# genjax-community/genjax

Measured on AMD Instinct MI355X. Metric: particle_steps_per_sec, higher is better.
Workload: dtype f32; 1 GPU; gmm_c8_d16 ImportanceK: propagate+reweight+LSE, systematic resample, gather (BASELINE.json configs[1]); k_particles_per_gpu=1048576, k_particles_total=1048576, rng_stream=flat, exchange=none

## Files before the change

### genjax_amd/csrc/gjx_resample.hip

```cpp
#include <math.h>
#include <string.h>

#include "gjx_device.h"
#include "gjx_host.h"
#include "gjx_scan.h"
#include "gjx_tile.h"

namespace gjx {

struct PickPair {
  float v;
  int32_t i;
};

GJX_DEV void pick_better(float& v, int32_t& i, float ov, int32_t oi) {
  if (ov > v || (ov == v && oi < i)) { v = ov; i = oi; }
}

template <int RNG>
__global__ __launch_bounds__(256) void k_pick_partial(const float* logw, int64_t K, int64_t offset, const float* lse,
                                                     key2 key, PickPair* partials) {
  __shared__ float rv[4];
  __shared__ int32_t ri[4];
  const float l = lse[2];
  float bv = -INFINITY;
  int32_t bi = 0x7FFFFFFF;
  for (int64_t i = (int64_t)blockIdx.x * 256 + threadIdx.x; i < K; i += (int64_t)gridDim.x * 256) {
    const uint64_t gi = (uint64_t)(offset + i);
    uint32_t bits;
    if (RNG == GJX_RNG_JAX32) {
      const key2 h = fold_in64(key, gi);
      bits = h.a ^ h.b;
    } else {
      const key2 h = fold_in64(key, gi >> 1);
      bits = (gi & 1u) ? h.b : h.a;
    }
    const float v = (logw[i] - l) + gumbel_from_bits(bits);
    pick_better(bv, bi, v, (int32_t)gi);
  }
#pragma unroll
  for (int o = 32; o > 0; o >>= 1) {
    const float ov = __shfl_xor(bv, o, 64);
    const int32_t oi = __shfl_xor(bi, o, 64);
    pick_better(bv, bi, ov, oi);
  }
  if ((threadIdx.x & 63) == 0) { rv[threadIdx.x >> 6] = bv; ri[threadIdx.x >> 6] = bi; }
  __syncthreads();
  if (threadIdx.x == 0) {
    for (int w = 1; w < 4; ++w) pick_better(bv, bi, rv[w], ri[w]);
    partials[blockIdx.x] = PickPair{bv, bi};
  }
}

__global__ __launch_bounds__(256) void k_pick_finish(const PickPair* partials, int n, PickPair* out) {
  __shared__ float rv[4];
  __shared__ int32_t ri[4];
  float bv = -INFINITY;
// ... 182 lines not shown
        const int h = atomicAdd(&n_heavy, 1);
        h_i[h] = (int32_t)i; h_lo[h] = lo; h_hi[h] = hi;
      } else if (hi > lo) {
        if (ancestors) for (int64_t j = lo; j < hi; ++j) ancestors[j] = (int32_t)i;
        if (GATHER) {
          for (int r = 0; r < rows; ++r) {
            const float v = src[(int64_t)r * src_stride + i];
            for (int64_t j = lo; j < hi; ++j) dst[(int64_t)r * dst_stride + j] = v;
          }
        }
      }
    }
  }
  __syncthreads();
  const int nh = n_heavy;
  for (int h = 0; h < nh; ++h) {
    const int32_t pi = h_i[h];
    const int64_t lo = h_lo[h], hi = h_hi[h];
    if (ancestors) for (int64_t j = lo + threadIdx.x; j < hi; j += 256) ancestors[j] = pi;
    if (GATHER) {
      for (int r = 0; r < rows; ++r) {
        const float v = src[(int64_t)r * src_stride + pi];
        for (int64_t j = lo + threadIdx.x; j < hi; j += 256) dst[(int64_t)r * dst_stride + j] = v;
      }
    }
  }
}

template <int ITEMS>
__global__ __launch_bounds__(256) void k_resample_fused(const float* __restrict__ x, int64_t K, int mode,
                                                       const float* lse, int n_partials, float* lse_out,
                                                       float log_k_total, double u, int64_t N, int32_t* ancestors,
                                                       uint64_t* cum_out, uint64_t* base_total_out,
                                                       unsigned long long* agg, unsigned* ctrl) {
  __shared__ float fred[8];
  __shared__ ScanSmem sm;
  unsigned epoch;
  const unsigned long long tag = grid_tag(ctrl, &epoch);
  const int64_t i0 = ((int64_t)blockIdx.x * 256 + threadIdx.x) * ITEMS;
  float xv[ITEMS];
#pragma unroll
  for (int k = 0; k < ITEMS; ++k) xv[k] = (i0 + k < K) ? x[i0 + k] : 0.0f;
  float sm_sum;
  const float mx = block_ref_max(mode, lse, n_partials, fred, &sm_sum);
  if (mode == 2 && lse_out && blockIdx.x == 0 && threadIdx.x == 0) {
    const float l = mx > -INFINITY ? mx + logf(sm_sum) : -INFINITY;
    lse_out[0] = mx; lse_out[1] = sm_sum; lse_out[2] = l; lse_out[3] = l - log_k_total;
  }
  tile_scan_expand<ITEMS, false>(xv, mode, mx, i0, K, u, N, ancestors, cum_out, base_total_out, agg, tag, ctrl, epoch, true, sm);
}

constexpr int kGatherMaxTiles = 1024;

template <int ITEMS>
__global__ __launch_bounds__(256) void k_resample_gather(const float* __restrict__ x, int64_t K, int mode,
                                                        const float* lse, int n_partials, float* lse_out,
                                                        float log_k_total, double u, const float* __restrict__ src,
                                                        int64_t src_stride, int rows, float* __restrict__ dst,
                                                        int64_t dst_stride, int32_t* ancestors,
                                                        unsigned long long* agg, unsigned* ctrl,
                                                        unsigned long long* timeline) {
#define GJX_STAMP(n) do { if (timeline && threadIdx.x == 0) timeline[blockIdx.x * 8 + (n)] = __builtin_amdgcn_s_memrealtime(); } while (0)
  GJX_STAMP(0);
  constexpr int TILE = 256 * ITEMS;
  __shared__ float fred[8];
  __shared__ uint64_t wsum[4];
  __shared__ uint64_t P[kGatherMaxTiles + 1];
  constexpr int CH = 3;
  __shared__ uint64_t cumL[CH * TILE];
  __shared__ uint64_t s_wtot[CH][4];
  __shared__ int s_range[2];
  unsigned epoch;
  const unsigned long long tag = grid_tag(ctrl, &epoch);
  const int nb = (int)gridDim.x;
  const int lane = threadIdx.x & 63, wid = threadIdx.x >> 6;
  const int64_t i0 = ((int64_t)blockIdx.x * 256 + threadIdx.x) * ITEMS;
  auto load_tile = [&](int64_t p0, float (&v)[ITEMS]) {
    if (ITEMS == 4 && p0 + 4 <= K) {
      const float4 q4 = *(const float4*)(x + p0);
      v[0] = q4.x; v[1] = q4.y; v[2] = q4.z; v[3] = q4.w;
    } else {
#pragma unroll
      for (int k = 0; k < ITEMS; ++k) v[k] = (p0 + k < K) ? x[p0 + k] : 0.0f;
    }
  };
  const int w0 = (int)blockIdx.x - 1;
  float xv[ITEMS], xn[2][ITEMS];
  load_tile(i0, xv);
  float sm_sum;
  const float mx = block_ref_max(mode, lse, n_partials, fred, &sm_sum);
  if (mode == 2 && lse_out && blockIdx.x == 0 && threadIdx.x == 0) {
    const float l = mx > -INFINITY ? mx + logf(sm_sum) : -INFINITY;
    lse_out[0] = mx; lse_out[1] = sm_sum; lse_out[2] = l; lse_out[3] = l - log_k_total;
  }
  uint64_t qown[ITEMS], sown = 0, incown;
  {
#pragma unroll
    for (int k = 0; k < ITEMS; ++k) { sown += (i0 + k < K) ? weight_q(xv, k, mode, mx) : 0; qown[k] = sown; }
    incown = wave_scan_u64(sown);
    if (lane == 63) { wsum[wid] = incown; s_wtot[1][wid] = incown; }
    __syncthreads();
    if (threadIdx.x == 0) grid_publish(agg, tag, wsum[0] + wsum[1] + wsum[2] + wsum[3]);
  }
  GJX_STAMP(1);
#pragma unroll
  for (int c = 0; c < 2; ++c) {
    const int tc = w0 + 2 * c;
#pragma unroll
    for (int k = 0; k < ITEMS; ++k) xn[c][k] = 0.0f;
    if (tc >= 0 && tc < nb) load_tile((int64_t)tc * TILE + (int64_t)threadIdx.x * ITEMS, xn[c]);
  }
  {
    uint64_t qn[2][ITEMS], sn[2], incn[2];
#pragma unroll
// ... 131 lines not shown
        inc[c] = sacc[c];
      }
#pragma unroll
      for (int c = 0; c < CH; ++c) inc[c] = wave_scan_u64(inc[c]);
      if (lane == 63) {
#pragma unroll
        for (int c = 0; c < CH; ++c) s_wtot[c][wid] = inc[c];
      }
      __syncthreads();
#pragma unroll
      for (int c = 0; c < CH; ++c) {
        uint64_t base = P[tsrc[c]] + (inc[c] - sacc[c]);
        for (int w = 0; w < wid; ++w) base += s_wtot[c][w];
#pragma unroll
        for (int k = 0; k < ITEMS; ++k) cumL[c * TILE + threadIdx.x * ITEMS + k] = base + qi[c][k];
      }
      __syncthreads();
      int pos[ITEMS];
      const uint64_t* cm[ITEMS];
      bool mine[ITEMS];
#pragma unroll
      for (int k = 0; k < ITEMS; ++k) {
        mine[k] = kpos[k] >= idx && kpos[k] < idx + CH;
        cm[k] = cumL + (mine[k] ? (kpos[k] - idx) * TILE : 0);
        pos[k] = 0;
      }
#pragma unroll
      for (int q = TILE >> 2; q >= 1; q >>= 2) {
#pragma unroll
        for (int k = 0; k < ITEMS; ++k) {
          const uint64_t pa = cm[k][pos[k] + q - 1], pb = cm[k][pos[k] + 2 * q - 1], pc = cm[k][pos[k] + 3 * q - 1];
          pos[k] += (pa <= T[k] ? q : 0) + (pb <= T[k] ? q : 0) + (pc <= T[k] ? q : 0);
        }
      }
#pragma unroll
      for (int k = 0; k < ITEMS; ++k)
        if (mine[k]) anc[k] = (int32_t)((int64_t)tile[k] * TILE + pos[k]);
      idx = nidx;
    }
    }
  }
  GJX_STAMP(4);
#pragma unroll
  for (int k = 0; k < ITEMS; ++k) anc[k] = max(0, min(anc[k], (int32_t)(K - 1)));
  const bool whole = i0 + ITEMS <= K;
  if (ancestors) {
    if (ITEMS == 4 && whole) *(int4*)(ancestors + i0) = make_int4(anc[0], anc[1], anc[2], anc[3]);
    else {
#pragma unroll
      for (int k = 0; k < ITEMS; ++k) if (i0 + k < K) ancestors[i0 + k] = anc[k];
    }
  }
  const bool vec = ITEMS == 4 && whole && (dst_stride & 3) == 0 && (((uintptr_t)dst) & 15) == 0;
  if (vec) {
#pragma unroll 4
    for (int r = 0; r < rows; ++r) {
      const float* sr = src + (int64_t)r * src_stride;
      float4 v;
      v.x = sr[anc[0]]; v.y = sr[anc[ITEMS > 1 ? 1 : 0]]; v.z = sr[anc[ITEMS > 2 ? 2 : 0]]; v.w = sr[anc[ITEMS > 3 ? 3 : 0]];
      *(float4*)(dst + (int64_t)r * dst_stride + i0) = v;
    }
  } else {
#pragma unroll 4
    for (int r = 0; r < rows; ++r) {
      const float* sr = src + (int64_t)r * src_stride;
#pragma unroll
      for (int k = 0; k < ITEMS; ++k) if (i0 + k < K) dst[(int64_t)r * dst_stride + i0 + k] = sr[anc[k]];
    }
  }
  GJX_STAMP(5);
#undef GJX_STAMP
}

constexpr int kGatherTiledMaxTiles = 65536;

template <bool GATED>
__global__ __launch_bounds__(kTileQ) void k_tile_totals(const float* __restrict__ logw, int64_t K, uint64_t* S, int32_t* E, const int32_t* gate) {
  constexpr int NW = kTileQ / 64;
  if (GATED && *gate == 0) return;
  __shared__ float fred[NW];
  __shared__ uint64_t wsum[NW];
  const int lane = threadIdx.x & 63, wid = threadIdx.x >> 6;
  const int64_t i = (int64_t)blockIdx.x * kTileQ + threadIdx.x;
  const float lw = i < K ? logw[i] : -INFINITY;
  const float wm = wave_max(lw);
  if (lane == 0) fred[wid] = wm;
  __syncthreads();
  float bm = fred[0];
#pragma unroll
  for (int w = 1; w < NW; ++w) bm = fmaxf(bm, fred[w]);
  const int e = tile_exponent(bm);
  const uint64_t tot_w = wave_total_u64(i < K ? tile_q(lw, e) : 0);
  if (lane == 0) wsum[wid] = tot_w;
  __syncthreads();
  if (threadIdx.x == 0) {
    uint64_t tot = 0;
    for (int w = 0; w < NW; ++w) tot += wsum[w];
    S[blockIdx.x] = tot;
    E[blockIdx.x] = tot ? e : kTileDead;
  }
}

template <int ITEMS, bool PLANNED, bool GATED>
__global__ __launch_bounds__(256) void k_resample_gather_tiled(const float* __restrict__ x, int64_t K, const uint64_t* __restrict__ S,
                                                              const int32_t* __restrict__ E, const uint64_t* __restrict__ Pg,
                                                              const int32_t* __restrict__ shg, int lse_mode, const float* lse,
                                                              int n_partials, float* lse_out, float log_k_total, double u,
                                                              const float* __restrict__ src, int64_t src_stride, int rows,
                                                              float* __restrict__ dst, int64_t dst_stride, int32_t* ancestors,
                                                              unsigned* ctrl, unsigned long long* timeline, const int32_t* gate) {
#define GJX_STAMP(n) do { if (timeline && threadIdx.x == 0) timeline[blockIdx.x * 8 + (n)] = __builtin_amdgcn_s_memrealtime(); } while (0)
  GJX_STAMP(0);
  static_assert(ITEMS == 4, "a block consumes one quantisation tile: 256 lanes x 4 slots");
  extern __shared__ __align__(16) unsigned char gt_dyn[];
  const int nt = (int)gridDim.x;
  uint64_t* const Pl = (uint64_t*)gt_dyn;
  int32_t* const Ebl = (int32_t*)(Pl + ((nt + 2) & ~1));
  __shared__ TiledSearchShared sh;
  const int64_t i0 = ((int64_t)blockIdx.x * 256 + threadIdx.x) * ITEMS;
  int32_t anc[ITEMS];
  if (GATED && *gate == 0) {
#pragma unroll
    for (int k = 0; k < ITEMS; ++k) anc[k] = (int32_t)((i0 + k < K) ? i0 + k : K - 1);
  } else
  tiled_search_tile<PLANNED>(x, K, S, E, Pg, shg, nt, (int)blockIdx.x, Pl, Ebl, sh, lse_mode, lse, n_partials, lse_out, log_k_total, u, ctrl, timeline, anc);
  GJX_STAMP(4);
  const bool whole = i0 + ITEMS <= K;
  if (ancestors) {
    if (whole) *(int4*)(ancestors + i0) = make_int4(anc[0], anc[1], anc[2], anc[3]);
    else {
#pragma unroll
      for (int k = 0; k < ITEMS; ++k) if (i0 + k < K) ancestors[i0 + k] = anc[k];
    }
  }
  const bool vec = whole && (dst_stride & 3) == 0 && (((uintptr_t)dst) & 15) == 0;
  if (vec) {
#pragma unroll 4
    for (int r = 0; r < rows; ++r) {
      const float* sr = src + (int64_t)r * src_stride;
      float4 v;
      v.x = sr[anc[0]]; v.y = sr[anc[1]]; v.z = sr[anc[2]]; v.w = sr[anc[3]];
      *(float4*)(dst + (int64_t)r * dst_stride + i0) = v;
    }
  } else {
#pragma unroll 4
    for (int r = 0; r < rows; ++r) {
      const float* sr = src + (int64_t)r * src_stride;
#pragma unroll
      for (int k = 0; k < ITEMS; ++k) if (i0 + k < K) dst[(int64_t)r * dst_stride + i0 + k] = sr[anc[k]];
    }
  }
  GJX_STAMP(5);
#undef GJX_STAMP
}

__global__ __launch_bounds__(256) void k_multinomial(const uint64_t* cum, int64_t K, const uint64_t* base_total,
                                                    key2 key, int64_t out_begin, int64_t n_out, int32_t* ancestors) {
  const int64_t j = (int64_t)blockIdx.x * 256 + threadIdx.x;
  if (j >= n_out) return;
  const uint64_t base = base_total[0], total = base_total[1];
  const key2 h = fold_in64(key, (uint64_t)(out_begin + j));
  const uint64_t r = (((uint64_t)h.a << 32) | h.b) >> 11;
  const double uj = (double)r * (1.0 / 9007199254740992.0);
  const uint64_t T = (uint64_t)(uj * (double)total);
  int32_t a = -1;
  if (K > 0) {
    const uint64_t local = cum[K - 1];
    if (T >= base && T < base + local) a = (int32_t)upper_search(cum, K, T - base);
  }
  ancestors[j] = a;
}

__global__ __launch_bounds__(256) void k_gather_rows(const float* __restrict__ src, int64_t src_stride,
                                                    const int32_t* __restrict__ anc, int64_t n_out, int rows,
                                                    float* __restrict__ dst, int64_t dst_stride) {
  const int64_t j = (int64_t)blockIdx.x * 256 + threadIdx.x;
  if (j >= n_out) return;
  const int32_t a = anc[j];
  if ((uint64_t)(int64_t)a >= (uint64_t)src_stride) return;
  for (int r = 0; r < rows; ++r) dst[(int64_t)r * dst_stride + j] = src[(int64_t)r * src_stride + a];
}


int launch_expand_planned(const uint64_t* cum, int64_t K, const gjx_shard_plan* plan_dev, double u, int64_t N_total,
                          int32_t* ancestors, int64_t anc_capacity, hipStream_t st) {
  const uint64_t* bt = reinterpret_cast<const uint64_t*>(plan_dev);
  const int64_t* range = reinterpret_cast<const int64_t*>(plan_dev) + 2;
  hipLaunchKernelGGL(k_systematic_expand<false>, dim3((unsigned)((K + 255) / 256)), dim3(256), 0, st, cum, K, bt, u, N_total,
                     (int64_t)0, anc_capacity, ancestors, (const float*)nullptr, (int64_t)0, 0, (float*)nullptr, (int64_t)0,
                     range);
  GJX_CHECK_LAUNCH("gjx_shard_resample(expand)");
  return GJX_OK;
}

struct EssArgs {
  const float* inc;
  float* W;
  float* w_copy;
  int64_t K;
  const int32_t* fresh;
  unsigned long long* pm;
  unsigned* p2;
  unsigned* ticket;
  float* out4;
// ... 157 lines not shown
  GJX_CHECK_LAUNCH("gjx_categorical_pick/partial");
  hipLaunchKernelGGL(k_pick_finish, dim3(1), dim3(256), 0, st, (const PickPair*)partials, nblocks, (PickPair*)out_dev);
  GJX_CHECK_LAUNCH("gjx_categorical_pick/finish");
  return GJX_OK;
}

extern "C" int gjx_trials_lse_pick(const float* logw, int64_t n_trials, int64_t K, int64_t particle_offset, uint32_t key0, uint32_t key1,
                                   int32_t rng_mode, float* lse_out, int32_t* pick_out, void* stream) {
  if (!logw || !lse_out || n_trials <= 0 || K <= 0 || n_trials > 0x7fffffffLL || particle_offset < 0 ||
      (pick_out && particle_offset + n_trials * K > 0x7fffffffLL))
    return gjx_fail(GJX_EINVAL, "gjx_trials_lse_pick: bad argument");
  hipStream_t st = (hipStream_t)stream;
  const float log_k = (float)log((double)K);
  if (rng_mode == GJX_RNG_JAX32)
    hipLaunchKernelGGL(k_trials_lse_pick<GJX_RNG_JAX32>, dim3((unsigned)n_trials), dim3(256), 0, st, logw, K, particle_offset, key2{key0, key1},
                       pick_out ? 1 : 0, log_k, lse_out, pick_out);
  else
    hipLaunchKernelGGL(k_trials_lse_pick<GJX_RNG_FLAT>, dim3((unsigned)n_trials), dim3(256), 0, st, logw, K, particle_offset, key2{key0, key1},
                       pick_out ? 1 : 0, log_k, lse_out, pick_out);
  GJX_CHECK_LAUNCH("gjx_trials_lse_pick");
  return GJX_OK;
}

extern "C" int gjx_weight_cumsum(const float* x, int64_t K, int32_t is_log, const float* lse, int32_t n_partials,
                                 uint64_t* cum, uint64_t* base_total_dev, float* lse_out, int64_t K_total,
                                 void* workspace, size_t workspace_bytes, void* stream) {
  if (!x || !cum || !base_total_dev || K <= 0 || is_log < 0 || is_log > 2 || (is_log && !lse) || (is_log == 2 && n_partials <= 0))
    return gjx_fail(GJX_EINVAL, "gjx_weight_cumsum: bad argument");
  if (!workspace || workspace_bytes < gjx_workspace_bytes(GJX_OP_RESAMPLE, K)) return gjx_fail(GJX_EWORKSPACE, "gjx_weight_cumsum: workspace too small");
  hipStream_t st = (hipStream_t)stream;
  const int nblocks = (int)((K + kScanTile - 1) / kScanTile);
  uint64_t* bs = (uint64_t*)((char*)workspace + kWsHeaderBytes);
  const float log_k = (float)log((double)(K_total > 0 ? K_total : K));
  hipLaunchKernelGGL(k_wsum_blocks, dim3(nblocks), dim3(256), 0, st, x, K, (int)is_log, lse, (int)n_partials, lse_out, log_k, bs);
  GJX_CHECK_LAUNCH("gjx_weight_cumsum/sum");
  hipLaunchKernelGGL(k_wscan_write, dim3(nblocks), dim3(256), 0, st, x, K, (int)is_log, lse, (int)n_partials, (const uint64_t*)bs, cum, base_total_dev);
  GJX_CHECK_LAUNCH("gjx_weight_cumsum/write");
  return GJX_OK;
}

extern "C" int gjx_resample_systematic(const uint64_t* cum, int64_t K, const uint64_t* base_total_dev, double u,
                                       int64_t N_total, int64_t out_begin, int64_t n_out, int32_t* ancestors,
                                       void* stream) {
  if (!cum || !base_total_dev || !ancestors || K <= 0 || N_total <= 0 || n_out < 0 || !(u >= 0.0 && u < 1.0))
    return gjx_fail(GJX_EINVAL, "gjx_resample_systematic: bad argument");
  if (n_out == 0) return GJX_OK;
  hipLaunchKernelGGL(k_systematic_expand<false>, dim3((unsigned)((K + 255) / 256)), dim3(256), 0, (hipStream_t)stream, cum, K,
                     base_total_dev, u, N_total, out_begin, n_out, ancestors, (const float*)nullptr, (int64_t)0, 0,
                     (float*)nullptr, (int64_t)0);
  GJX_CHECK_LAUNCH("gjx_resample_systematic");
  return GJX_OK;
}

static int env_items() {
  const char* e = getenv("GJX_RESAMPLE_ITEMS");
  const int v = e ? atoi(e) : 0;
  return (v == 1 || v == 4 || v == 16) ? v : 0;
}

extern "C" int gjx_resample_indices(const float* x, int64_t K, int32_t is_log, const float* lse, int32_t n_partials,
                                    double u, int64_t N, int32_t* ancestors, uint64_t* cum, uint64_t* base_total_dev,
                                    float* lse_out, int64_t K_total, void* workspace, size_t workspace_bytes, void* stream) {
  if (!x || K <= 0 || N <= 0 || is_log < 0 || is_log > 2 || (is_log && !lse) || (is_log == 2 && n_partials <= 0) ||
      !(u >= 0.0 && u < 1.0) || (!ancestors && !cum))
    return gjx_fail(GJX_EINVAL, "gjx_resample_indices: bad argument");
  if (!workspace || workspace_bytes < gjx_workspace_bytes(GJX_OP_RESAMPLE, K)) return gjx_fail(GJX_EWORKSPACE, "gjx_resample_indices: workspace too small");
  int items = env_items();
  int64_t nblocks = 0;
  const int cand[3] = {1, 4, 16};
  bool fits = false;
  for (int c = 0; c < 3 && !fits; ++c) {
    if (items && cand[c] != items) continue;
    const void* fn = cand[c] == 1 ? (const void*)k_resample_fused<1> : cand[c] == 4 ? (const void*)k_resample_fused<4> : (const void*)k_resample_fused<16>;
    const int cap = gjx_coresident_blocks(fn, 256, 0);
    nblocks = (K + 256 * (int64_t)cand[c] - 1) / (256 * (int64_t)cand[c]);
    if (nblocks <= cap) { items = cand[c]; fits = true; }
  }
  hipStream_t st = (hipStream_t)stream;
  if (!fits || !ancestors) {
    if (!cum || !base_total_dev) return gjx_fail(GJX_EUNSUPPORTED, "gjx_resample_indices: the grid would not be co-resident on this device and there are no cum/base_total buffers for the three-launch path");
    int rc = gjx_weight_cumsum(x, K, is_log, lse, n_partials, cum, base_total_dev, lse_out, K_total, workspace, workspace_bytes, stream);
    if (rc || !ancestors) return rc;
    return gjx_resample_systematic(cum, K, base_total_dev, u, N, 0, N, ancestors, stream);
  }
  unsigned* ctrl = (unsigned*)workspace + 8;
  unsigned long long* agg = (unsigned long long*)((char*)workspace + kWsHeaderBytes);
  const float log_k = (float)log((double)(K_total > 0 ? K_total : K));
#define GJX_RF(IT) hipLaunchKernelGGL((k_resample_fused<IT>), dim3((unsigned)nblocks), dim3(256), 0, st, x, K, (int)is_log, lse, \
                                      (int)n_partials, lse_out, log_k, u, N, ancestors, cum, base_total_dev, agg, ctrl)
  if (items == 1) GJX_RF(1); else if (items == 4) GJX_RF(4); else GJX_RF(16);
#undef GJX_RF
  GJX_CHECK_LAUNCH("gjx_resample_indices");
  return GJX_OK;
}

extern "C" int gjx_resample_gather(const float* x, int64_t K, int32_t is_log, const float* lse, int32_t n_partials, double u,
                                   const float* src, int64_t src_stride, int32_t rows, float* dst, int64_t dst_stride,
                                   int32_t* ancestors, float* lse_out, int64_t K_total, void* workspace,
                                   size_t workspace_bytes, void* stream) {
  if (!x || K <= 0 || is_log < 0 || is_log > 2 || (is_log && !lse) || (is_log == 2 && n_partials <= 0) ||
      !(u >= 0.0 && u < 1.0) || rows < 0 || (rows > 0 && (!src || !dst)) || K > 0x7fffffffLL)
    return gjx_fail(GJX_EINVAL, "gjx_resample_gather: bad argument");
  if (!workspace || workspace_bytes < gjx_workspace_bytes(GJX_OP_RESAMPLE, K)) return gjx_fail(GJX_EWORKSPACE, "gjx_resample_gather: workspace too small");
  int items = 0;
  int64_t nblocks = 0;
  const int cand[2] = {1, 4};
  const int forced = env_items();
  for (int c = 0; c < 2 && !items; ++c) {
    if (forced && cand[c] != forced) continue;
    const void* fn = cand[c] == 1 ? (const void*)k_resample_gather<1> : (const void*)k_resample_gather<4>;
    const int cap = gjx_coresident_blocks(fn, 256, 0);
    nblocks = (K + 256 * (int64_t)cand[c] - 1) / (256 * (int64_t)cand[c]);
    if (nblocks <= cap && nblocks <= kGatherMaxTiles) items = cand[c];
  }
  if (!items) return gjx_fail(GJX_EUNSUPPORTED, "gjx_resample_gather: K is too large for one co-resident grid on this device (use gjx_resample_indices + gjx_gather_rows)");
  hipStream_t st = (hipStream_t)stream;
  unsigned* ctrl = (unsigned*)workspace + 8;
  unsigned long long* agg = (unsigned long long*)((char*)workspace + kWsHeaderBytes);
  const float log_k = (float)log((double)(K_total > 0 ? K_total : K));
  unsigned long long* timeline = nullptr;
  timeline = gjx::debug_timeline(64 * (size_t)nblocks);
#define GJX_RG(IT) hipLaunchKernelGGL((k_resample_gather<IT>), dim3((unsigned)nblocks), dim3(256), 0, st, x, K, (int)is_log, lse, \
                                      (int)n_partials, lse_out, log_k, u, src, src_stride, (int)rows, dst, dst_stride, ancestors, agg, ctrl, timeline)
  if (items == 1) GJX_RG(1); else GJX_RG(4);
#undef GJX_RG
  GJX_CHECK_LAUNCH("gjx_resample_gather");
  return GJX_OK;
}

int gjx::resample_gather_tiled_gated(const float* logw, int64_t K, const uint64_t* tile_S, const int32_t* tile_E, int32_t lse_mode,
                                     const float* lse, int32_t n_partials, double u, const float* src, int64_t src_stride,
                                     int32_t rows, float* dst, int64_t dst_stride, int32_t* ancestors, float* lse_out,
                                     int64_t K_total, void* workspace, size_t workspace_bytes, void* stream, const int32_t* gate) {
  if (!logw || K <= 0 || !(u >= 0.0 && u < 1.0) || rows < 0 || (rows > 0 && (!src || !dst)) || K > 0x7fffffffLL ||
      (lse_mode != 0 && lse_mode != 2) || (lse_mode == 2 && (!lse || n_partials <= 0)) || ((tile_S == nullptr) != (tile_E == nullptr)))
    return gjx_fail(GJX_EINVAL, "gjx_resample_gather_tiled: bad argument");
  const int64_t nt = (K + kTileQ - 1) / kTileQ;
  if (nt > kGatherTiledMaxTiles) return gjx_fail(GJX_EUNSUPPORTED, "gjx_resample_gather_tiled: more than 65536 tiles (K > 2^26): use gjx_resample_indices_tiled + gjx_gather_rows");
  if (!workspace || workspace_bytes < gjx_workspace_bytes(GJX_OP_RESAMPLE, K) || kWsHeaderBytes + 12 * (size_t)nt > workspace_bytes)
    return gjx_fail(GJX_EWORKSPACE, "gjx_resample_gather_tiled: workspace too small");
  hipStream_t st = (hipStream_t)stream;
  unsigned* ctrl = (unsigned*)workspace + 8;
  if (!tile_S) {
    uint64_t* S = (uint64_t*)((char*)workspace + kWsHeaderBytes);
    int32_t* E = (int32_t*)(S + nt);
    if (gate) hipLaunchKernelGGL(k_tile_totals<true>, dim3((unsigned)nt), dim3(kTileQ), 0, st, logw, K, S, E, gate);
    else hipLaunchKernelGGL(k_tile_totals<false>, dim3((unsigned)nt), dim3(kTileQ), 0, st, logw, K, S, E, (const int32_t*)nullptr);
    GJX_CHECK_LAUNCH("gjx_resample_gather_tiled/totals");
    tile_S = S; tile_E = E;
  }
  const float log_k = (float)log((double)(K_total > 0 ? K_total : K));
  unsigned long long* timeline = gjx::debug_timeline(64 * (size_t)nt);
  if (nt > 1024 || getenv("GJX_TILED_PLANNED")) {
    uint64_t* Pg = (uint64_t*)((char*)workspace + kWsHeaderBytes + 12 * (size_t)nt + 16);
    Pg = (uint64_t*)(((uintptr_t)Pg + 15) & ~(uintptr_t)15);
    int32_t* shg = (int32_t*)(Pg + nt + 1);
    if ((char*)(shg + nt) > (char*)workspace + workspace_bytes) return gjx_fail(GJX_EWORKSPACE, "gjx_resample_gather_tiled: workspace too small");
    const int rc = gjx::launch_tiled_plan(tile_S, tile_E, (int)nt, Pg, shg, ctrl, st, gate);
    if (rc) return rc;
#define GJX_GT(GATED) hipLaunchKernelGGL((k_resample_gather_tiled<4, true, GATED>), dim3((unsigned)nt), dim3(256), 0, st, logw, K, tile_S, tile_E, \
                       (const uint64_t*)Pg, (const int32_t*)shg, (int)lse_mode, lse, (int)n_partials, lse_out, log_k, u, src, src_stride, (int)rows, \
                       dst, dst_stride, ancestors, ctrl, timeline, gate)
    if (gate) GJX_GT(true); else GJX_GT(false);
#undef GJX_GT
  } else {
    const size_t lds = 8 * (size_t)((nt + 2) & ~1) + 4 * (size_t)nt;
#define GJX_GT(GATED) hipLaunchKernelGGL((k_resample_gather_tiled<4, false, GATED>), dim3((unsigned)nt), dim3(256), lds, st, logw, K, tile_S, tile_E, \
                       (const uint64_t*)nullptr, (const int32_t*)nullptr, (int)lse_mode, lse, (int)n_partials, lse_out, log_k, u, src, src_stride, \
                       (int)rows, dst, dst_stride, ancestors, ctrl, timeline, gate)
    if (gate) GJX_GT(true); else GJX_GT(false);
#undef GJX_GT
  }
  GJX_CHECK_LAUNCH("gjx_resample_gather_tiled");
  return GJX_OK;
}

extern "C" int gjx_resample_gather_tiled(const float* logw, int64_t K, const uint64_t* tile_S, const int32_t* tile_E, int32_t lse_mode,
                                         const float* lse, int32_t n_partials, double u, const float* src, int64_t src_stride,
                                         int32_t rows, float* dst, int64_t dst_stride, int32_t* ancestors, float* lse_out,
                                         int64_t K_total, void* workspace, size_t workspace_bytes, void* stream) {
  return gjx::resample_gather_tiled_gated(logw, K, tile_S, tile_E, lse_mode, lse, n_partials, u, src, src_stride, rows, dst, dst_stride, ancestors,
                                          lse_out, K_total, workspace, workspace_bytes, stream, nullptr);
}

extern "C" int gjx_resample_gather_systematic(const uint64_t* cum, int64_t K, const uint64_t* base_total_dev, double u,
                                              int64_t N_total, int64_t out_begin, int64_t n_out, const float* src,
                                              int64_t src_stride, int32_t rows, float* dst, int64_t dst_stride,
                                              int32_t* ancestors, void* stream) {
  if (!cum || !base_total_dev || !src || !dst || !ancestors || K <= 0 || N_total <= 0 || n_out < 0 || rows < 0 ||
      !(u >= 0.0 && u < 1.0))
    return gjx_fail(GJX_EINVAL, "gjx_resample_gather_systematic: bad argument");
  if (n_out == 0) return GJX_OK;
  const int rc = gjx_resample_systematic(cum, K, base_total_dev, u, N_total, out_begin, n_out, ancestors, stream);
  if (rc) return rc;
  return gjx_gather_rows(src, src_stride, ancestors, n_out, rows, dst, dst_stride, stream);
}

extern "C" int gjx_resample_multinomial(const uint64_t* cum, int64_t K, const uint64_t* base_total_dev,
                                        uint32_t key0, uint32_t key1, int64_t N_total, int64_t out_begin,
                                        int64_t n_out, int32_t* ancestors, void* stream) {
  (void)N_total;
  if (!cum || !base_total_dev || !ancestors || K <= 0 || n_out < 0) return gjx_fail(GJX_EINVAL, "gjx_resample_multinomial: bad argument");
  if (n_out == 0) return GJX_OK;
  hipLaunchKernelGGL(k_multinomial, dim3((unsigned)((n_out + 255) / 256)), dim3(256), 0, (hipStream_t)stream, cum, K,
                     base_total_dev, key2{key0, key1}, out_begin, n_out, ancestors);
  GJX_CHECK_LAUNCH("gjx_resample_multinomial");
  return GJX_OK;
}

extern "C" int gjx_gather_rows(const float* src, int64_t src_stride, const int32_t* anc, int64_t n_out, int32_t rows,
                               float* dst, int64_t dst_stride, void* stream) {
  if (!src || !anc || !dst || n_out < 0 || rows < 0) return gjx_fail(GJX_EINVAL, "gjx_gather_rows: bad argument");
  if (n_out == 0 || rows == 0) return GJX_OK;
  hipLaunchKernelGGL(k_gather_rows, dim3((unsigned)((n_out + 255) / 256)), dim3(256), 0, (hipStream_t)stream, src,
                     src_stride, anc, n_out, (int)rows, dst, dst_stride);
  GJX_CHECK_LAUNCH("gjx_gather_rows");
  return GJX_OK;
}


extern "C" int gjx_ess(const float* logw, int64_t K, float* out4, void* workspace, size_t workspace_bytes, void* stream) {
  if (!logw || !out4 || K <= 0 || K > (int64_t)1 << 31) return gjx_fail(GJX_EINVAL, "gjx_ess: bad argument");
  const int64_t nt = (K + kTileQ - 1) / kTileQ;
// ... 10 lines not shown
```

### profiles/microbench/gather_tiled_timeline.py

```python
import os, sys, time, torch, numpy as np
sys.path.insert(0, os.path.dirname(os.path.dirname(os.path.dirname(os.path.abspath(__file__)))))
from genjax_amd import kernels, workloads, _abi as A
K = 1 << 20
prog, _ = workloads.gmm_program()
ws = kernels.workspace(A.OP_RUN, K, "cuda"); ws2 = kernels.workspace(A.OP_RESAMPLE, K, "cuda")
out = kernels.run_program(prog, (0, 1), K, ws=ws, want_weight=False, want_lse=False, want_tiles=True)
part = out["_partials"]; print("tiles offset", part.tiles, "n partials", part.count())
rows = torch.empty_like(out["choices"]); lse = torch.empty(4, device="cuda")
def step_old():
    kernels.run_program(prog, (0, 2), K, ws=ws, out=out, want_weight=False, want_lse=False)
    kernels.resample_gather(out["logw"], 0.37, out["choices"], partials=(ws, part.count()), lse_out=lse, out=rows, ws=ws2, allow_fallback=False)
def step_new():
    kernels.run_program(prog, (0, 2), K, ws=ws, out=out, want_weight=False, want_lse=False, want_tiles=True)
    kernels.resample_gather_tiled(out["logw"], 0.37, out["choices"], partials=(ws, part.count()), tiles=part.tiles, lse_out=lse, out=rows, ws=ws2)
def step_new_notiles():
    kernels.run_program(prog, (0, 2), K, ws=ws, out=out, want_weight=False, want_lse=False)
    kernels.resample_gather_tiled(out["logw"], 0.37, out["choices"], partials=(ws, part.count()), tiles=0, lse_out=lse, out=rows, ws=ws2)
for name, fn in (("old", step_old), ("tiled+tiles", step_new), ("tiled no tiles", step_new_notiles), ("old", step_old), ("tiled+tiles", step_new)):
    for _ in range(50): fn()
    torch.cuda.synchronize(); t0 = time.perf_counter()
    for _ in range(400): fn()
    torch.cuda.synchronize(); print(name, "us/step %.2f" % ((time.perf_counter() - t0) / 400 * 1e6), "lse", lse.tolist()[2:])
tl = torch.zeros((1024, 8), dtype=torch.int64, device="cuda")
from genjax_amd._lib import load as _load
import ctypes as _C
_load().gjx_debug_timeline(_C.c_void_p(tl.data_ptr()), tl.numel() * tl.element_size())
step_new(); torch.cuda.synchronize()
t = tl.cpu().numpy().astype(np.float64); t0 = t[:, 0].min()
for j, n in [(0, "start"), (1, "totals read, Emax"), (2, "prefix"), (3, "tiles found + window cum"), (4, "ancestors known"), (5, "rows copied (end)")]:
    c = (t[:, j] - t0) * 0.01
    print(f"{n:26s} min {c.min():7.2f}  median {np.median(c):7.2f}  max {c.max():7.2f} us")
```

### profiles/microbench/gather_timeline.py

```python
import os, sys, torch, numpy as np
sys.path.insert(0, os.path.dirname(os.path.dirname(os.path.dirname(os.path.abspath(__file__)))))
from genjax_amd import kernels, workloads, _abi as A
K = 1 << 20
prog, _ = workloads.gmm_program()
ws = kernels.workspace(A.OP_RUN, K, "cuda"); ws2 = kernels.workspace(A.OP_RESAMPLE, K, "cuda")
out = kernels.run_program(prog, (0, 1), K, ws=ws, want_weight=False, want_lse=False)
n_part = kernels.run_partials_count(prog, K, 0)
rows = torch.empty_like(out["choices"]); lse = torch.empty(4, device="cuda")
def go():
    kernels.run_program(prog, (0, 2), K, ws=ws, out=out, want_weight=False, want_lse=False)
    kernels.resample_gather(out["logw"], 0.37, out["choices"], partials=(ws, n_part), lse_out=lse, out=rows, ws=ws2, allow_fallback=False)
for _ in range(20): go()
tl = torch.zeros((1024, 8), dtype=torch.int64, device="cuda")
from genjax_amd._lib import load as _load
import ctypes as _C
_load().gjx_debug_timeline(_C.c_void_p(tl.data_ptr()), tl.numel() * tl.element_size())
go(); torch.cuda.synchronize()
t = tl.cpu().numpy().astype(np.float64); t0 = t[:, 0].min()
for j, n in [(0, "start"), (1, "tile total published"), (2, "totals gathered"), (6, "prefix of totals"), (7, "source tiles found"), (3, "tile list known"), (4, "ancestors known"), (5, "rows copied (end)")]:
    c = (t[:, j] - t0) * 0.01
    print(f"{n:24s} min {c.min():7.2f}  median {np.median(c):7.2f}  max {c.max():7.2f} us")
```

Baseline: 18.41 billion particle-steps/s.

## Stage gathered rows through LDS with coalesced float4 loads when ancestors are clustered

Adds a staged row-copy path for the resample gather kernels. When every lane in a wave has ancestors that fall inside a 512-float window, the wave reads that window with coalesced float4 loads, parks it in LDS (reusing the cumL scratch), and then picks the ancestor values from LDS. This replaces four scattered dword gathers per row. Waves whose ancestors are spread wider fall back to the direct gather. The path is on by default (env GJX_GATHER_STAGED) and adds a block barrier plus LDS traffic before the copy.

```diff
diff --git a/genjax_amd/csrc/gjx_resample.hip b/genjax_amd/csrc/gjx_resample.hip
--- a/genjax_amd/csrc/gjx_resample.hip
+++ b/genjax_amd/csrc/gjx_resample.hip
@@ -3,6 +3,7 @@
 
 #include "gjx_device.h"
 #include "gjx_host.h"
+#include "gjx_rowcopy.h"
 #include "gjx_scan.h"
 #include "gjx_tile.h"
 
@@ -291,14 +292,15 @@
 
 constexpr int kGatherMaxTiles = 1024;
 
-template <int ITEMS>
+template <int ITEMS, bool STAGED>
 __global__ __launch_bounds__(256) void k_resample_gather(const float* __restrict__ x, int64_t K, int mode,
                                                         const float* lse, int n_partials, float* lse_out,
                                                         float log_k_total, double u, const float* __restrict__ src,
                                                         int64_t src_stride, int rows, float* __restrict__ dst,
                                                         int64_t dst_stride, int32_t* ancestors,
                                                         unsigned long long* agg, unsigned* ctrl,
-                                                        unsigned long long* timeline) {
+                                                        unsigned long long* timeline, unsigned long long* copy_stamp) {
+  static_assert(!STAGED || ITEMS == 4, "the staged copy is written for 4 slots per lane");
 #define GJX_STAMP(n) do { if (timeline && threadIdx.x == 0) timeline[blockIdx.x * 8 + (n)] = __builtin_amdgcn_s_memrealtime(); } while (0)
   GJX_STAMP(0);
   constexpr int TILE = 256 * ITEMS;
@@ -536,22 +538,16 @@
     }
   }
   const bool vec = ITEMS == 4 && whole && (dst_stride & 3) == 0 && (((uintptr_t)dst) & 15) == 0;
-  if (vec) {
-#pragma unroll 4
-    for (int r = 0; r < rows; ++r) {
-      const float* sr = src + (int64_t)r * src_stride;
-      float4 v;
-      v.x = sr[anc[0]]; v.y = sr[anc[ITEMS > 1 ? 1 : 0]]; v.z = sr[anc[ITEMS > 2 ? 2 : 0]]; v.w = sr[anc[ITEMS > 3 ? 3 : 0]];
-      *(float4*)(dst + (int64_t)r * dst_stride + i0) = v;
-    }
-  } else {
-#pragma unroll 4
-    for (int r = 0; r < rows; ++r) {
-      const float* sr = src + (int64_t)r * src_stride;
-#pragma unroll
-      for (int k = 0; k < ITEMS; ++k) if (i0 + k < K) dst[(int64_t)r * dst_stride + i0 + k] = sr[anc[k]];
-    }
-  }
+  bool copied = false;
+  if constexpr (STAGED) {
+    static_assert(4 * kCopySliceFloats * sizeof(float) <= sizeof(cumL), "the staging slices live in cumL");
+    __syncthreads();
+    if (copy_stamp && threadIdx.x == 0) copy_stamp[blockIdx.x] = __builtin_amdgcn_s_memrealtime();
+    const bool aligned = (src_stride & 3) == 0 && (((uintptr_t)src) & 15) == 0;
+    copied = copy_rows_staged<kCopySixRows>(src, src_stride, rows, dst, dst_stride, K, i0, anc, vec && aligned,
+                                                     (float*)cumL + wid * kCopySliceFloats);
+  }
+  if (!copied) copy_rows_direct<ITEMS>(src, src_stride, rows, dst, dst_stride, K, i0, anc, vec);
   GJX_STAMP(5);
 #undef GJX_STAMP
 }
@@ -585,7 +581,7 @@
   }
 }
 
-template <int ITEMS, bool PLANNED, bool GATED>
+template <int ITEMS, bool PLANNED, bool GATED, bool STAGED>
 __global__ __launch_bounds__(256) void k_resample_gather_tiled(const float* __restrict__ x, int64_t K, const uint64_t* __restrict__ S,
                                                               const int32_t* __restrict__ E, const uint64_t* __restrict__ Pg,
                                                               const int32_t* __restrict__ shg, int lse_mode, const float* lse,
@@ -618,22 +614,16 @@
     }
   }
   const bool vec = whole && (dst_stride & 3) == 0 && (((uintptr_t)dst) & 15) == 0;
-  if (vec) {
-#pragma unroll 4
-    for (int r = 0; r < rows; ++r) {
-      const float* sr = src + (int64_t)r * src_stride;
-      float4 v;
-      v.x = sr[anc[0]]; v.y = sr[anc[1]]; v.z = sr[anc[2]]; v.w = sr[anc[3]];
-      *(float4*)(dst + (int64_t)r * dst_stride + i0) = v;
-    }
-  } else {
-#pragma unroll 4
-    for (int r = 0; r < rows; ++r) {
-      const float* sr = src + (int64_t)r * src_stride;
-#pragma unroll
-      for (int k = 0; k < ITEMS; ++k) if (i0 + k < K) dst[(int64_t)r * dst_stride + i0 + k] = sr[anc[k]];
-    }
-  }
+  bool copied = false;
+  if constexpr (STAGED) {
+    static_assert(4 * kCopySliceFloats * sizeof(float) <= sizeof(sh.cumL), "the staging slices live in sh.cumL");
+    __syncthreads();
+    GJX_STAMP(6);
+    const bool aligned = (src_stride & 3) == 0 && (((uintptr_t)src) & 15) == 0;
+    copied = copy_rows_staged<kCopySixRows>(src, src_stride, rows, dst, dst_stride, K, i0, anc, vec && aligned,
+                                                     (float*)sh.cumL + (threadIdx.x >> 6) * kCopySliceFloats);
+  }
+  if (!copied) copy_rows_direct<ITEMS>(src, src_stride, rows, dst, dst_stride, K, i0, anc, vec);
   GJX_STAMP(5);
 #undef GJX_STAMP
 }
@@ -897,6 +887,11 @@
   return GJX_OK;
 }
 
+static bool env_gather_staged() {
+  const char* e = getenv("GJX_GATHER_STAGED");
+  return !(e && e[0] == '0');
+}
+
 static int env_items() {
   const char* e = getenv("GJX_RESAMPLE_ITEMS");
   const int v = e ? atoi(e) : 0;
@@ -951,9 +946,11 @@
   int64_t nblocks = 0;
   const int cand[2] = {1, 4};
   const int forced = env_items();
+  const bool staged = env_gather_staged();
   for (int c = 0; c < 2 && !items; ++c) {
     if (forced && cand[c] != forced) continue;
-    const void* fn = cand[c] == 1 ? (const void*)k_resample_gather<1> : (const void*)k_resample_gather<4>;
+    const void* fn = cand[c] == 1 ? (const void*)k_resample_gather<1, false>
+                                  : staged ? (const void*)k_resample_gather<4, true> : (const void*)k_resample_gather<4, false>;
     const int cap = gjx_coresident_blocks(fn, 256, 0);
     nblocks = (K + 256 * (int64_t)cand[c] - 1) / (256 * (int64_t)cand[c]);
     if (nblocks <= cap && nblocks <= kGatherMaxTiles) items = cand[c];
@@ -965,9 +962,12 @@
   const float log_k = (float)log((double)(K_total > 0 ? K_total : K));
   unsigned long long* timeline = nullptr;
   timeline = gjx::debug_timeline(64 * (size_t)nblocks);
-#define GJX_RG(IT) hipLaunchKernelGGL((k_resample_gather<IT>), dim3((unsigned)nblocks), dim3(256), 0, st, x, K, (int)is_log, lse, \
-                                      (int)n_partials, lse_out, log_k, u, src, src_stride, (int)rows, dst, dst_stride, ancestors, agg, ctrl, timeline)
-  if (items == 1) GJX_RG(1); else GJX_RG(4);
+  unsigned long long* copy_stamp = gjx::debug_timeline(72 * (size_t)nblocks);
+  if (copy_stamp) copy_stamp += 8 * (size_t)nblocks;
+#define GJX_RG(IT, ST) hipLaunchKernelGGL((k_resample_gather<IT, ST>), dim3((unsigned)nblocks), dim3(256), 0, st, x, K, (int)is_log, lse, \
+                                          (int)n_partials, lse_out, log_k, u, src, src_stride, (int)rows, dst, dst_stride, ancestors, agg, ctrl, \
+                                          timeline, copy_stamp)
+  if (items == 1) GJX_RG(1, false); else if (staged) GJX_RG(4, true); else GJX_RG(4, false);
 #undef GJX_RG
   GJX_CHECK_LAUNCH("gjx_resample_gather");
   return GJX_OK;
@@ -996,6 +996,7 @@
   }
   const float log_k = (float)log((double)(K_total > 0 ? K_total : K));
   unsigned long long* timeline = gjx::debug_timeline(64 * (size_t)nt);
+  const bool staged = env_gather_staged();
   if (nt > 1024 || getenv("GJX_TILED_PLANNED")) {
     uint64_t* Pg = (uint64_t*)((char*)workspace + kWsHeaderBytes + 12 * (size_t)nt + 16);
     Pg = (uint64_t*)(((uintptr_t)Pg + 15) & ~(uintptr_t)15);
@@ -1003,17 +1004,19 @@
     if ((char*)(shg + nt) > (char*)workspace + workspace_bytes) return gjx_fail(GJX_EWORKSPACE, "gjx_resample_gather_tiled: workspace too small");
     const int rc = gjx::launch_tiled_plan(tile_S, tile_E, (int)nt, Pg, shg, ctrl, st, gate);
     if (rc) return rc;
-#define GJX_GT(GATED) hipLaunchKernelGGL((k_resample_gather_tiled<4, true, GATED>), dim3((unsigned)nt), dim3(256), 0, st, logw, K, tile_S, tile_E, \
+#define GJX_GT(GATED, ST) hipLaunchKernelGGL((k_resample_gather_tiled<4, true, GATED, ST>), dim3((unsigned)nt), dim3(256), 0, st, logw, K, tile_S, tile_E, \
                        (const uint64_t*)Pg, (const int32_t*)shg, (int)lse_mode, lse, (int)n_partials, lse_out, log_k, u, src, src_stride, (int)rows, \
                        dst, dst_stride, ancestors, ctrl, timeline, gate)
-    if (gate) GJX_GT(true); else GJX_GT(false);
+    if (gate) { if (staged) GJX_GT(true, true); else GJX_GT(true, false); }
+    else { if (staged) GJX_GT(false, true); else GJX_GT(false, false); }
 #undef GJX_GT
   } else {
     const size_t lds = 8 * (size_t)((nt + 2) & ~1) + 4 * (size_t)nt;
-#define GJX_GT(GATED) hipLaunchKernelGGL((k_resample_gather_tiled<4, false, GATED>), dim3((unsigned)nt), dim3(256), lds, st, logw, K, tile_S, tile_E, \
+#define GJX_GT(GATED, ST) hipLaunchKernelGGL((k_resample_gather_tiled<4, false, GATED, ST>), dim3((unsigned)nt), dim3(256), lds, st, logw, K, tile_S, tile_E, \
                        (const uint64_t*)nullptr, (const int32_t*)nullptr, (int)lse_mode, lse, (int)n_partials, lse_out, log_k, u, src, src_stride, \
                        (int)rows, dst, dst_stride, ancestors, ctrl, timeline, gate)
-    if (gate) GJX_GT(true); else GJX_GT(false);
+    if (gate) { if (staged) GJX_GT(true, true); else GJX_GT(true, false); }
+    else { if (staged) GJX_GT(false, true); else GJX_GT(false, false); }
 #undef GJX_GT
   }
   GJX_CHECK_LAUNCH("gjx_resample_gather_tiled");
diff --git a/genjax_amd/csrc/gjx_rowcopy.h b/genjax_amd/csrc/gjx_rowcopy.h
--- /dev/null
+++ b/genjax_amd/csrc/gjx_rowcopy.h
@@ -0,0 +1,104 @@
+#pragma once
+#include <stdint.h>
+
+#ifndef GJX_DEV
+#define GJX_DEV __device__ __forceinline__
+#endif
+
+namespace gjx {
+
+constexpr int kCopySpan = 512;
+constexpr int kCopyDepth = 3;
+constexpr int kCopySliceFloats = kCopyDepth * kCopySpan;
+constexpr bool kCopySixRows = true;
+
+template <int ITEMS>
+GJX_DEV void copy_rows_direct(const float* __restrict__ src, int64_t src_stride, int rows, float* __restrict__ dst,
+                              int64_t dst_stride, int64_t K, int64_t i0, const int32_t (&anc)[ITEMS], bool vec) {
+  if (vec) {
+#pragma unroll 4
+    for (int r = 0; r < rows; ++r) {
+      const float* sr = src + (int64_t)r * src_stride;
+      float4 v;
+      v.x = sr[anc[0]]; v.y = sr[anc[ITEMS > 1 ? 1 : 0]]; v.z = sr[anc[ITEMS > 2 ? 2 : 0]]; v.w = sr[anc[ITEMS > 3 ? 3 : 0]];
+      *(float4*)(dst + (int64_t)r * dst_stride + i0) = v;
+    }
+  } else {
+#pragma unroll 4
+    for (int r = 0; r < rows; ++r) {
+      const float* sr = src + (int64_t)r * src_stride;
+#pragma unroll
+      for (int k = 0; k < ITEMS; ++k) if (i0 + k < K) dst[(int64_t)r * dst_stride + i0 + k] = sr[anc[k]];
+    }
+  }
+}
+
+template <bool TWO, bool SIX>
+GJX_DEV void copy_rows_staged_loop(const float* __restrict__ src, int64_t src_stride, int rows, float* __restrict__ dst,
+                                   int64_t dst_stride, int64_t i0, int64_t q0, int64_t q1, const unsigned (&off)[4], float* slice) {
+  static_assert(kCopyDepth == 3, "the groups are written out for three LDS rows (plain float4 values, so that they stay in registers)");
+  constexpr bool HALVES = !TWO && SIX;
+  constexpr int G = HALVES ? 6 : 3;
+  constexpr int HALF = kCopySpan / 2;
+  const int w = 4 * (threadIdx.x & 63);
+  auto row = [&](int r) { return src + (int64_t)(r < rows ? r : rows - 1) * src_stride; };
+  auto fetch = [&](int r, float4& a, float4& b) {
+    a = *(const float4*)(row(r) + q0);
+    if (TWO) b = *(const float4*)(row(r) + q1);
+    else if (SIX) b = *(const float4*)(row(r + 3) + q0);
+  };
+  auto park = [&](int d, const float4& a, const float4& b) {
+    *(float4*)(slice + d * kCopySpan + w) = a;
+    if (TWO || SIX) *(float4*)(slice + d * kCopySpan + HALF + w) = b;
+  };
+  auto pick = [&](const float* s, int r) {
+    float4 v;
+    v.x = s[off[0]]; v.y = s[off[1]]; v.z = s[off[2]]; v.w = s[off[3]];
+    *(float4*)(dst + (int64_t)r * dst_stride + i0) = v;
+  };
+#define GJX_GROUP(r0, full) do {                                                                          \
+    float4 a0, a1, a2, b0, b1, b2;                                                                        \
+    b0 = b1 = b2 = make_float4(0.f, 0.f, 0.f, 0.f);                                                       \
+    fetch((r0), a0, b0); fetch((r0) + 1, a1, b1); fetch((r0) + 2, a2, b2);                                \
+    park(0, a0, b0);                                                                                      \
+    if ((full) || (r0) + 1 < rows) park(1, a1, b1);                                                       \
+    if ((full) || (r0) + 2 < rows) park(2, a2, b2);                                                       \
+    __builtin_amdgcn_wave_barrier();                                                                      \
+    _Pragma("unroll") for (int d = 0; d < 3; ++d) {                                                       \
+      if ((full) || (r0) + d < rows) pick(slice + d * kCopySpan, (r0) + d);                               \
+      if (HALVES && ((full) || (r0) + 3 + d < rows)) pick(slice + d * kCopySpan + HALF, (r0) + 3 + d);    \
+    }                                                                                                     \
+    __builtin_amdgcn_wave_barrier();                                                                      \
+  } while (0)
+  int r = 0;
+  for (; r + G <= rows; r += G) GJX_GROUP(r, true);
+  if (r < rows) GJX_GROUP(r, false);
+#undef GJX_GROUP
+}
+
+template <bool SIX>
+GJX_DEV bool copy_rows_staged(const float* __restrict__ src, int64_t src_stride, int rows, float* __restrict__ dst,
+                              int64_t dst_stride, int64_t K, int64_t i0, const int32_t (&anc)[4], bool eligible, float* slice) {
+  const int lane = threadIdx.x & 63;
+  const int32_t lo4 = __builtin_amdgcn_readfirstlane(anc[0]) & ~3;
+  const int32_t hi = __builtin_amdgcn_readlane(anc[3], 63);
+  unsigned off[4];
+  bool ok = eligible;
+#pragma unroll
+  for (int k = 0; k < 4; ++k) {
+    off[k] = (unsigned)(anc[k] - lo4);
+    ok = ok && off[k] < (unsigned)kCopySpan && anc[k] <= hi && (int64_t)(anc[k] | 3) < K;
+  }
+  if (__builtin_amdgcn_ballot_w64(ok) != ~0ull) return false;
+  const bool two = hi - lo4 >= kCopySpan / 2;
+  const int64_t hi4 = hi & ~3;
+  const int64_t p0 = (int64_t)lo4 + 4 * lane, p1 = p0 + kCopySpan / 2;
+  const int64_t q0 = p0 < hi4 ? p0 : hi4, q1 = p1 < hi4 ? p1 : hi4;
+  if (rows > 0) {
+    if (two) copy_rows_staged_loop<true, SIX>(src, src_stride, rows, dst, dst_stride, i0, q0, q1, off, slice);
+    else copy_rows_staged_loop<false, SIX>(src, src_stride, rows, dst, dst_stride, i0, q0, q1, off, slice);
+  }
+  return true;
+}
+
+}
diff --git a/profiles/microbench/copy_bound.hip b/profiles/microbench/copy_bound.hip
--- /dev/null
+++ b/profiles/microbench/copy_bound.hip
@@ -0,0 +1,122 @@
+#include <hip/hip_runtime.h>
+#include <hip/hip_ext.h>
+#include <stdio.h>
+#include <stdlib.h>
+#include <string.h>
+#include <algorithm>
+#include <vector>
+
+#include "gjx_rowcopy.h"
+
+#define CK(x) do { hipError_t e_ = (x); if (e_ != hipSuccess) { printf("HIP error %s at %s:%d\n", hipGetErrorString(e_), __FILE__, __LINE__); exit(1); } } while (0)
+
+constexpr int64_t K = 1 << 20;
+constexpr int R = 17;
+constexpr int NB = (int)(K / 1024);
+struct Shape { int64_t K, src_stride, dst_stride; int rows; };
+
+__global__ __launch_bounds__(256) void k_fill(float* src, unsigned salt) {
+  const int64_t n4 = (int64_t)R * K / 4;
+  for (int64_t i = (int64_t)blockIdx.x * 256 + threadIdx.x; i < n4; i += (int64_t)gridDim.x * 256) {
+    const unsigned h = (unsigned)i * 2654435761u + salt;
+    ((float4*)src)[i] = make_float4((float)(h & 0xffff), (float)(h >> 16), (float)((h >> 8) & 0xffff), (float)(i & 0xffff));
+  }
+}
+
+__global__ __launch_bounds__(256) void k_plain(const float* __restrict__ src, float* __restrict__ dst, const int32_t* anc_dev, Shape s) {
+  const int64_t i0 = ((int64_t)blockIdx.x * 256 + threadIdx.x) * 4;
+#pragma unroll 4
+  for (int r = 0; r < s.rows; ++r) *(float4*)(dst + (int64_t)r * s.dst_stride + i0) = *(const float4*)(src + (int64_t)r * s.src_stride + i0);
+}
+
+__global__ __launch_bounds__(256) void k_gather(const float* __restrict__ src, float* __restrict__ dst, const int32_t* anc_dev, Shape s) {
+  const int64_t i0 = ((int64_t)blockIdx.x * 256 + threadIdx.x) * 4;
+  const int4 q = *(const int4*)(anc_dev + i0);
+  const int32_t anc[4] = {q.x, q.y, q.z, q.w};
+  gjx::copy_rows_direct<4>(src, s.src_stride, s.rows, dst, s.dst_stride, s.K, i0, anc, true);
+}
+
+template <bool SIX>
+__global__ __launch_bounds__(256) void k_staged(const float* __restrict__ src, float* __restrict__ dst, const int32_t* anc_dev, Shape s) {
+  __shared__ __align__(16) float lds[4 * gjx::kCopySliceFloats];
+  const int64_t i0 = ((int64_t)blockIdx.x * 256 + threadIdx.x) * 4;
+  const int4 q = *(const int4*)(anc_dev + i0);
+  const int32_t anc[4] = {q.x, q.y, q.z, q.w};
+  if (!gjx::copy_rows_staged<SIX>(src, s.src_stride, s.rows, dst, s.dst_stride, s.K, i0, anc, true, lds + (threadIdx.x >> 6) * gjx::kCopySliceFloats))
+    gjx::copy_rows_direct<4>(src, s.src_stride, s.rows, dst, s.dst_stride, s.K, i0, anc, true);
+}
+
+typedef void (*kern_t)(const float*, float*, const int32_t*, Shape);
+
+struct Stat { double med, lo, hi; };
+
+static Stat time_kernel(kern_t kern, float* src, float* dst, const int32_t* anc, int n) {
+  hipEvent_t e0, e1;
+  CK(hipEventCreate(&e0)); CK(hipEventCreate(&e1));
+  std::vector<double> us;
+  for (int it = 0; it < n + 3; ++it) {
+    hipLaunchKernelGGL(k_fill, dim3(2048), dim3(256), 0, 0, src, (unsigned)it);
+    hipExtLaunchKernelGGL(kern, dim3(NB), dim3(256), 0, 0, e0, e1, 0, (const float*)src, dst, anc, Shape{K, K, K, R});
+    CK(hipEventSynchronize(e1));
+    float ms = 0;
+    CK(hipEventElapsedTime(&ms, e0, e1));
+    if (it >= 3) us.push_back(ms * 1e3);
+  }
+  CK(hipEventDestroy(e0)); CK(hipEventDestroy(e1));
+  std::sort(us.begin(), us.end());
+  return Stat{us[us.size() / 2], us.front(), us.back()};
+}
+
+int main(int argc, char** argv) {
+  const char* anc_file = argc > 1 && argv[1][0] ? argv[1] : nullptr;
+  const int n = argc > 2 ? std::max(20, atoi(argv[2])) : 40;
+  float *src, *dst, *ref;
+  int32_t* anc;
+  const size_t bytes = (size_t)R * K * 4;
+  CK(hipMalloc(&src, bytes)); CK(hipMalloc(&dst, bytes)); CK(hipMalloc(&ref, bytes)); CK(hipMalloc(&anc, K * 4));
+  std::vector<int32_t> ident(K), real;
+  for (int64_t j = 0; j < K; ++j) ident[j] = (int32_t)j;
+  if (anc_file) {
+    FILE* f = fopen(anc_file, "rb");
+    real.resize(K);
+    if (!f || fread(real.data(), 4, K, f) != (size_t)K) { printf("cannot read %lld int32 from %s\n", (long long)K, anc_file); return 1; }
+    fclose(f);
+    for (int64_t j = 0; j < K; ++j)
+      if (real[j] < 0 || real[j] >= K) { printf("ancestor %d at slot %lld is outside the rows\n", real[j], (long long)j); return 1; }
+  }
+  struct Var { const char* name; kern_t k; };
+  const Var staged[2] = {{"(c) staged, 3 rows per group", k_staged<false>}, {"(c) staged, 6 when span < 256", k_staged<true>}};
+  auto line = [&](const char* name, const char* set, Stat s, const char* note) {
+    printf("%-30s %-9s median %6.2f  min %6.2f  max %6.2f us   %5.2f TB/s%s\n", name, set, s.med, s.lo, s.hi, 2.0 * bytes / s.med * 1e-6, note);
+    fflush(stdout);
+  };
+  printf("K = %lld, R = %d, %d blocks x 256, %d launches each, source filled before every launch (%.1f + %.1f MB)\n", (long long)K, R, NB, n,
+         bytes * 1e-6, bytes * 1e-6);
+  line("(a) plain float4 copy", "-", time_kernel(k_plain, src, dst, anc, n), "");
+  std::vector<float> h0(bytes / 4), h1(bytes / 4);
+  for (int set = 0; set < (anc_file ? 2 : 1); ++set) {
+    const std::vector<int32_t>& A = set ? real : ident;
+    const char* sname = set ? "real" : "identity";
+    CK(hipMemcpy(anc, A.data(), K * 4, hipMemcpyHostToDevice));
+    if (set) {
+      int64_t wide = 0;
+      for (int64_t w = 0; w < K / 256; ++w) {
+        const int32_t lo4 = A[w * 256] & ~3;
+        bool ok = true;
+        for (int j = 0; j < 256; ++j) ok = ok && (unsigned)(A[w * 256 + j] - lo4) < (unsigned)gjx::kCopySpan;
+        wide += !ok;
+      }
+      printf("real ancestors: %lld of %lld waves wider than the span (direct loop)\n", (long long)wide, (long long)(K / 256));
+    }
+    line("(b) 4 dword gathers", sname, time_kernel(k_gather, src, ref, anc, n), "");
+    CK(hipMemcpy(h0.data(), ref, bytes, hipMemcpyDeviceToHost));
+    for (const Var& v : staged) {
+      CK(hipMemset(dst, 0xff, bytes));
+      const Stat s = time_kernel(v.k, src, dst, anc, n);
+      CK(hipMemcpy(h1.data(), dst, bytes, hipMemcpyDeviceToHost));
+      line(v.name, sname, s, memcmp(h0.data(), h1.data(), bytes) ? "   ROWS DIFFER FROM (b)" : "   rows == (b)");
+    }
+    line("(a) plain float4 copy again", "-", time_kernel(k_plain, src, dst, anc, n), "");
+  }
+  return 0;
+}
diff --git a/profiles/microbench/copy_bound.py b/profiles/microbench/copy_bound.py
--- /dev/null
+++ b/profiles/microbench/copy_bound.py
@@ -0,0 +1,34 @@
+import os, subprocess, sys, tempfile
+import torch
+HERE = os.path.dirname(os.path.abspath(__file__))
+ROOT = os.path.dirname(os.path.dirname(HERE))
+sys.path.insert(0, ROOT)
+from genjax_amd import kernels, workloads, _abi as A
+
+exe = os.path.join(HERE, "build", "copy_bound")
+src = os.path.join(HERE, "copy_bound.hip")
+if not os.path.exists(exe) or os.path.getmtime(exe) < os.path.getmtime(src):
+    os.makedirs(os.path.dirname(exe), exist_ok=True)
+    subprocess.check_call([os.environ.get("HIPCC", "/opt/rocm/bin/hipcc"), "-O3", "-std=c++17", "--offload-arch=gfx950",
+                           "-I", os.path.join(ROOT, "genjax_amd", "csrc"), src, "-o", exe])
+K = 1 << 20
+prog, _ = workloads.gmm_program()
+ws = kernels.workspace(A.OP_RUN, K, "cuda"); ws2 = kernels.workspace(A.OP_RESAMPLE, K, "cuda")
+out = kernels.run_program(prog, (0, 1), K, ws=ws, want_weight=False, want_lse=False)
+n_part = kernels.run_partials_count(prog, K, 0)
+rows = torch.empty_like(out["choices"]); lse = torch.empty(4, device="cuda")
+anc = torch.empty(K, dtype=torch.int32, device="cuda")
+kernels.run_program(prog, (0, 2), K, ws=ws, out=out, want_weight=False, want_lse=False)
+kernels.resample_gather(out["logw"], 0.37, out["choices"], partials=(ws, n_part), lse_out=lse, out=rows, anc=anc, ws=ws2, allow_fallback=False)
+torch.cuda.synchronize()
+kernels.workspace_status(ws2)
+assert torch.equal(rows, out["choices"].index_select(1, anc.long()))
+a = anc.cpu()
+d = (a[1:] - a[:-1]).long()
+print("step: rows", tuple(rows.shape), " distinct ancestors %d of %d, largest jump %d" % (int(torch.unique(a).numel()), K, int(d.max())), flush=True)
+with tempfile.TemporaryDirectory() as tmp:
+    path = os.path.join(tmp, "ancestors.i32")
+    a.numpy().tofile(path)
+    del out, rows, anc, ws, ws2
+    torch.cuda.empty_cache()
+    sys.exit(subprocess.call([exe, path] + sys.argv[1:2]))
diff --git a/profiles/microbench/gather_tiled_timeline.py b/profiles/microbench/gather_tiled_timeline.py
--- a/profiles/microbench/gather_tiled_timeline.py
+++ b/profiles/microbench/gather_tiled_timeline.py
@@ -27,6 +27,9 @@
 _load().gjx_debug_timeline(_C.c_void_p(tl.data_ptr()), tl.numel() * tl.element_size())
 step_new(); torch.cuda.synchronize()
 t = tl.cpu().numpy().astype(np.float64); t0 = t[:, 0].min()
-for j, n in [(0, "start"), (1, "totals read, Emax"), (2, "prefix"), (3, "tiles found + window cum"), (4, "ancestors known"), (5, "rows copied (end)")]:
+for j, n in [(0, "start"), (1, "totals read, Emax"), (2, "prefix"), (3, "tiles found + window cum"), (4, "ancestors known"), (6, "copy starts (staged)"), (5, "rows copied (end)")]:
+    if j == 6 and not t[:, 6].any(): continue
     c = (t[:, j] - t0) * 0.01
     print(f"{n:26s} min {c.min():7.2f}  median {np.median(c):7.2f}  max {c.max():7.2f} us")
+c = (t[:, 5] - t[:, 4]) * 0.01
+print(f"{'copy phase per block':26s} min {c.min():7.2f}  median {np.median(c):7.2f}  max {c.max():7.2f} us   (ancestors known -> rows copied)")
diff --git a/profiles/microbench/gather_timeline.py b/profiles/microbench/gather_timeline.py
--- a/profiles/microbench/gather_timeline.py
+++ b/profiles/microbench/gather_timeline.py
@@ -11,12 +11,15 @@
     kernels.run_program(prog, (0, 2), K, ws=ws, out=out, want_weight=False, want_lse=False)
     kernels.resample_gather(out["logw"], 0.37, out["choices"], partials=(ws, n_part), lse_out=lse, out=rows, ws=ws2, allow_fallback=False)
 for _ in range(20): go()
-tl = torch.zeros((1024, 8), dtype=torch.int64, device="cuda")
+tl = torch.zeros(1024 * 9, dtype=torch.int64, device="cuda")
 from genjax_amd._lib import load as _load
 import ctypes as _C
 _load().gjx_debug_timeline(_C.c_void_p(tl.data_ptr()), tl.numel() * tl.element_size())
 go(); torch.cuda.synchronize()
-t = tl.cpu().numpy().astype(np.float64); t0 = t[:, 0].min()
-for j, n in [(0, "start"), (1, "tile total published"), (2, "totals gathered"), (6, "prefix of totals"), (7, "source tiles found"), (3, "tile list known"), (4, "ancestors known"), (5, "rows copied (end)")]:
+t = tl.cpu().numpy().astype(np.float64); t = np.concatenate([t[:8192].reshape(1024, 8), t[8192:].reshape(1024, 1)], axis=1); t0 = t[:, 0].min()
+for j, n in [(0, "start"), (1, "tile total published"), (2, "totals gathered"), (6, "prefix of totals"), (7, "source tiles found"), (3, "tile list known"), (4, "ancestors known"), (8, "copy starts (staged)"), (5, "rows copied (end)")]:
+    if j == 8 and not t[:, 8].any(): continue
     c = (t[:, j] - t0) * 0.01
     print(f"{n:24s} min {c.min():7.2f}  median {np.median(c):7.2f}  max {c.max():7.2f} us")
+c = (t[:, 5] - t[:, 4]) * 0.01
+print(f"{'copy phase per block':24s} min {c.min():7.2f}  median {np.median(c):7.2f}  max {c.max():7.2f} us   (ancestors known -> rows copied)")
```

Result: no change. 18.50 billion particle-steps/s (median of 3 runs) (+0.5%).
